# tim-speed/flexdiffuse

Measured on AMD Instinct MI355X. Metric: 512x512 50-step images/sec/node (SD1.5, batch=8/GPU, Linear image guidance), higher is better.
Workload: dtype fp16; 1 GPU; SD1.5 512x512 50-step DDIM + linear image guidance, CFG 8, batch=8/GPU (BASELINE configs[1]); parallelism=seed-sharded x1, preset=sd15, guidance=linear, img2img=False, unet_evaluations_per_image=50, launch=graph, scheduler=ddim

## Files before the change

### flexdiffuse_amd/csrc/norm.hip

```cpp
#include <stdlib.h>

#include "common.h"
#include "gn_slab.h"

#define GN_MAX_CHUNKS 256

__global__ void k_gn_stats(const half_t* __restrict__ x, float* __restrict__ part, int HW, int C,
                           int G, int PL, int pix_per_chunk, int ldx) {
    extern __shared__ float sm[];
    const int b = blockIdx.y, chunk = blockIdx.x;
    const int c8 = C >> 3;
    const int tid = threadIdx.x;
    const int cc = tid % c8, pl = tid / c8;
    const int p0 = chunk * pix_per_chunk;
    const int p1 = min(HW, p0 + pix_per_chunk);
    float s[8], q[8];
#pragma unroll
    for (int k = 0; k < 8; ++k) s[k] = q[k] = 0.f;
    if (pl < PL) {
        const half_t* base = x + ((size_t)b * HW) * ldx + cc * 8;
        int p = p0 + pl;
        uint4 raw[4], nxt[4];
        bool have = p + 3 * PL < p1;
        if (have) {
// ... 402 lines not shown
    FD_CHECK_LAUNCH("k_gn_stats/k_gn_apply");
    return FD_OK;
}

extern "C" int fd_groupnorm_apply_parts_f16(const void* x, int ldx, void* y, const float* gamma, const float* beta, const float* parts,
                                            int chunks, int B, int HW, int C, int G, float eps, int silu, void* stream) {
    FD_PLAN(fd_groupnorm_apply_parts_f16(x, ldx, y, gamma, beta, parts, chunks, B, HW, C, G, eps, silu, fd_s_));
    FD_CHECK_ARG(x && y && gamma && beta && parts, FD_EINVAL, "fd_groupnorm_apply_parts_f16: null pointer");
    FD_CHECK_ARG(B > 0 && HW > 0 && C > 0 && G > 0 && chunks > 0, FD_EINVAL, "fd_groupnorm_apply_parts_f16: bad dims");
    FD_CHECK_ARG(ldx >= C && ldx % 8 == 0 && (uintptr_t)x % 16 == 0 && C % 8 == 0 && C % G == 0 && G <= 64 && C / 8 <= 1024, FD_ESHAPE,
                 "fd_groupnorm_apply_parts_f16: ldx=%d >= C=%d, both multiples of 8, C a multiple of G=%d (G <= 64), x 16-byte aligned", ldx, C, G);
    FD_CHECK_ARG((long long)B * HW * ldx < 0x7fffffffLL, FD_ESHAPE, "fd_groupnorm_apply_parts_f16: tensor too large");
    hipStream_t st = (hipStream_t)stream;
    const int c8 = C / 8;
    int PL = 512 / c8;
    if (PL < 1) PL = 1;
    if (PL > HW) PL = HW;
    const int threads = ((c8 * PL + 63) / 64) * 64;
    int nchunk = 256 / B;
    if (nchunk < 1) nchunk = 1;
    if (nchunk > GN_MAX_CHUNKS) nchunk = GN_MAX_CHUNKS;
    int ppc = fd_cdiv(HW, nchunk);
    if (ppc < PL) ppc = PL;
    nchunk = fd_cdiv(HW, ppc);
    const size_t lds2 = (size_t)2 * threads * sizeof(double) + (size_t)2 * G * sizeof(float);
    fd_prof_begin(FD_FAMILY_GROUPNORM, st, (double)B * HW * C * 4.0, -1.0, fd_tag(13u, B, HW, C, ldx));
    hipLaunchKernelGGL(k_gn_apply, dim3(nchunk, B), dim3(threads), lds2, st, (const half_t*)x, (half_t*)y, parts, gamma, beta, HW, C, G,
                       chunks, PL, ppc, eps, silu, ldx);
    fd_prof_end(FD_FAMILY_GROUPNORM, st);
    FD_CHECK_LAUNCH("k_gn_apply");
    return FD_OK;
}

template <int VPL, int RPW, bool STATS = false>
__global__ __launch_bounds__(256) void k_layernorm(const half_t* __restrict__ x, void* __restrict__ y,
                                                   const float* __restrict__ gamma,
                                                   const float* __restrict__ beta, int rows, int C,
                                                   int ldx, int ldy, float eps, int out_f32) {
    const int lane = threadIdx.x & 63;
    const int row0 = (blockIdx.x * 4 + (threadIdx.x >> 6)) * RPW;
    if (row0 >= rows) return;
    half8 v[RPW][VPL];
#pragma unroll
    for (int r = 0; r < RPW; ++r) {
        const half_t* xr = x + (size_t)min(row0 + r, rows - 1) * ldx;
#pragma unroll
        for (int i = 0; i < VPL; ++i) {
            const int c = (lane + 64 * i) * 8;
            uint4 raw = make_uint4(0u, 0u, 0u, 0u);
            if (c < C) raw = *reinterpret_cast<const uint4*>(xr + c);
            v[r][i] = *reinterpret_cast<half8*>(&raw);
        }
    }
#pragma unroll
    for (int r = 0; r < RPW; ++r) {
        const int row = row0 + r;
        if (row >= rows) break;
        float sum = 0.f;
#pragma unroll
        for (int i = 0; i < VPL; ++i)
#pragma unroll
            for (int k = 0; k < 8; ++k) sum += (float)v[r][i][k];
        const float mean = fd_wave_sum(sum) / (float)C;
        float sq = 0.f;
#pragma unroll
        for (int i = 0; i < VPL; ++i) {
// ... 180 lines not shown
```

### flexdiffuse_amd/hip.py

```python
from __future__ import annotations

import ctypes
import os
from ctypes import c_char_p, c_double, c_float, c_int, c_int32, c_int64, c_uint64, c_void_p
from typing import Optional

import torch

_HERE = os.path.dirname(os.path.abspath(__file__))
LIB_PATH = os.environ.get('FD_LIB_PATH') or os.path.join(_HERE, 'libflexdiffuse_hip.so')

FD_OK, FD_EINVAL, FD_ESHAPE, FD_EHIP = 0, -1, -2, -3


class FDError(RuntimeError):
    '''HIP runtime failure reported by libflexdiffuse_hip.so (FD_EHIP).'''


class fd_tween_params(ctypes.Structure):
    _fields_ = [('threshold_floor', c_double), ('threshold_mult', c_double),
                ('clustered', c_double), ('max_guidance', c_double),
                ('header_max', c_double), ('order', c_int32), ('reuse', c_int32)]


P = c_void_p
_SIGNATURES = {
    'fd_abi_version': (c_int, []),
    'fd_last_error': (c_char_p, []),
    'fd_device_info': (c_int, [c_int, P, P, P, P, c_int]),
    'fd_prof_enable': (c_int, [c_int]),
    'fd_prof_set_stride': (c_int, [c_int]),
    'fd_prof_collect': (c_int, [c_int, P, P, P]),
    'fd_prof_collect2': (c_int, [c_int, P, P, P, P]),
    'fd_prof_calibrate': (c_int, [c_int, P, P]),
    'fd_prof_drain': (c_int, [P, P, P, P, P, c_int64, P]),
    'fd_guidance_workspace_floats': (c_int64, [c_int, c_int, c_int]),
    'fd_guidance_map': (c_int, [P, P, P, P, P, c_int, c_int, c_int, c_int, c_int, c_int, c_int, P]),
    'fd_guidance_tween': (c_int, [P, P, P, P, P, P, P, P, P, c_int, c_int, c_int, c_int, c_int,
                                  ctypes.POINTER(fd_tween_params), P]),
    'fd_guidance_concept_override': (c_int, [P, P, P, P, P, c_int, c_int, c_int, P]),
    'fd_guidance_header_pull': (c_int, [P, P, c_int, c_int, c_int, P]),
    'fd_gemm_f16': (c_int, [P, P]),
    'fd_gemm_can_emit_row_stats': (c_int, [c_int, c_int, c_int, c_int, c_int]),
    'fd_gemm_plan': (c_int, [c_void_p, c_void_p, c_void_p]),
    'fd_gemm_can_fuse_groupnorm': (c_int, [c_int, c_int, c_int, c_int, c_int]),
    'fd_gemm_gn_parts_chunks': (c_int, [P]),
    'fd_groupnorm_apply_parts_f16': (c_int, [P, c_int, P, P, P, P, c_int, c_int, c_int, c_int, c_int, c_float, c_int, P]),
    'fd_groupnorm_fold_linear_parts_f16': (c_int, [P, c_int, c_int, c_int, c_int, c_int, c_float, P, P, c_int, P, P, P]),
    'fd_attention_f16': (c_int, [P, P]),
    'fd_xattn_image_bytes': (c_int64, [c_int, c_int]),
    'fd_xattn_pack_kv_f16': (c_int, [P, P, P, P, c_int, c_int, c_int, c_int, c_int, c_int, c_int64, c_int64, P]),
    'fd_xattn_q_f16': (c_int, [P, P]),
    'fd_groupnorm_workspace_floats': (c_int64, [c_int, c_int]),
    'fd_groupnorm_nhwc_f16': (c_int, [P, P, P, P, P, c_int, c_int, c_int, c_int, c_float, c_int, P]),
    'fd_groupnorm_nhwc_ld_f16': (c_int, [P, c_int, P, P, P, P, c_int, c_int, c_int, c_int, c_float, c_int, P]),
    'fd_layernorm_f16': (c_int, [P, P, P, P, c_int, c_int, c_int, c_int, c_float, c_int, P]),
    'fd_ln_row_stats_f16': (c_int, [P, P, c_int, c_int, c_int, c_float, P]),
    'fd_ln_finalize_stats_f32': (c_int, [P, P, c_int, c_int, c_int, c_float, P]),
    'fd_groupnorm_fold_linear_f16': (c_int, [P, c_int, P, c_int, c_int, c_int, c_int, c_float, P, P, c_int, P, P, P]),
    'fd_softmax_rows_f16': (c_int, [P, c_int, c_int, c_int, c_float, P]),
    'fd_nchw_f32_to_nhwc_f16': (c_int, [P, P, c_int, c_int, c_int, c_int, c_int, c_float, P]),
    'fd_nhwc_f32_to_nchw_f32': (c_int, [P, P, c_int, c_int, c_int, c_int, c_float, c_float, c_int, P]),
    'fd_im2col_f16': (c_int, [P, P] + [c_int] * 12 + [P]),
    'fd_conv3x3_narrow_f16': (c_int, [P, P, P, P, c_int, P, c_int, c_int, c_int, c_int, c_int, c_int, c_int, c_float, P]),
    'fd_concat_channels_f16': (c_int, [P, P, P, c_int64, c_int, c_int, P]),
    'fd_cfg_ddim_step_f32': (c_int, [P, P, P, c_int, c_int, c_int, c_int, c_int, c_float, c_float,
                                     c_float, c_float, c_float, c_int, c_int, P]),
    'fd_axpby_f32': (c_int, [P, P, P, c_int64, c_float, c_float, c_int, P]),
    'fd_embed_tokens_f16': (c_int, [P, P, P, P, c_int, c_int, c_int, c_int, P]),
    'fd_vit_assemble_f16': (c_int, [P, P, P, P, c_int, c_int, c_int, P]),
    'fd_timestep_embedding_f16': (c_int, [P, c_int, P, c_int, c_int, P]),
    'fd_copy2d_f16': (c_int, [P, c_int, P, c_int, c_int64, c_int, P]),
    'fd_repeat_rows_f16': (c_int, [P, c_int, P, c_int, c_int64, c_int, c_int, P]),
    'fd_plan_create': (c_int, [P]),
    'fd_plan_destroy': (c_int, [P]),
    'fd_plan_record_begin': (c_int, [P]),
    'fd_plan_record_end': (c_int, [P]),
    'fd_plan_size': (c_int, [P, P]),
    'fd_plan_replay': (c_int, [P, P]),
    'fd_region_blend_f32': (c_int, [P, P] + [c_int] * 7 + [c_float, P]),
    'fd_composite_step_f32': (c_int, [P, P, P, P, c_int, c_int, c_int, c_int, c_int, c_int, c_float, c_float,
# ... 183 lines not shown
```

### flexdiffuse_amd/ops.py

```python
from __future__ import annotations

import ctypes
import os
from ctypes import c_float, c_int32, c_int64, c_void_p
from dataclasses import dataclass
from typing import Optional, Tuple

import torch

from . import hip

ACT_NONE, ACT_SILU, ACT_QUICK_GELU, ACT_GELU, ACT_GEGLU = 0, 1, 2, 3, 4
FAMILY_GEMM, FAMILY_ATTENTION, FAMILY_GROUPNORM, FAMILY_OTHER = 0, 1, 2, 3


class fd_gemm_desc(ctypes.Structure):
    _fields_ = [('A', c_void_p), ('W', c_void_p), ('C', c_void_p), ('bias', c_void_p),
                ('bias2', c_void_p), ('residual', c_void_p),
                ('M', c_int32), ('N', c_int32), ('K', c_int32),
                ('lda', c_int32), ('ldw', c_int32), ('ldc', c_int32), ('ldr', c_int32),
                ('ld_bias2', c_int32), ('rows_per_sample', c_int32), ('act', c_int32),
                ('out_f32', c_int32), ('alpha', c_float),
                ('conv', c_int32), ('in_h', c_int32), ('in_w', c_int32), ('in_c', c_int32),
                ('out_h', c_int32), ('out_w', c_int32), ('kh', c_int32), ('kw', c_int32),
# ... 739 lines not shown


_gn_ws = {}
_gn_ws_retired = []


def _gn_workspace(B: int, G: int, dev) -> torch.Tensor:
    n = hip.lib().fd_groupnorm_workspace_floats(B, G)
    key = (dev.index if dev.index is not None else 0, WS_SLOT)
    ws = _gn_ws.get(key)
    if ws is None or ws.numel() < n:
        if ws is not None:
            _gn_ws_retired.append(ws)
        ws = torch.empty(n, dtype=torch.float32, device=dev)
        _gn_ws[key] = ws
    return ws


def groupnorm(x: Act, gamma: torch.Tensor, beta: torch.Tensor, G: int, eps: float,
              silu: bool, parts: Optional['GNParts'] = None) -> Act:
    assert x.t.stride(1) == 1
    out = _empty(tuple(x.t.shape), torch.float16, x.t)
    if parts is not None:
        assert parts.G == G and parts.t.shape == (x.B, parts.chunks, G, 2)
        hip.call('fd_groupnorm_apply_parts_f16', x.t.data_ptr(), x.t.stride(0), out.data_ptr(), gamma.data_ptr(), beta.data_ptr(),
                 parts.t.data_ptr(), parts.chunks, x.B, x.HW, x.C, G, eps, int(silu), hip.stream())
        return Act(out, x.B, x.H, x.W)
    ws = _gn_workspace(x.B, G, x.t.device)
    hip.call('fd_groupnorm_nhwc_ld_f16', x.t.data_ptr(), x.t.stride(0), out.data_ptr(), gamma.data_ptr(),
             beta.data_ptr(), ws.data_ptr(), x.B, x.HW, x.C, G, eps, int(silu), hip.stream())
    return Act(out, x.B, x.H, x.W)


@dataclass
class GNFold:
    wg: torch.Tensor
    biasf: torch.Tensor
    G: int
    eps: float
    N: int
    C: int


def prep_gn_fold(w: torch.Tensor, b: Optional[torch.Tensor], gamma: torch.Tensor, beta: torch.Tensor, G: int, eps: float,
                 dev) -> GNFold:
    w = w.reshape(w.shape[0], -1).float()
    N, C = w.shape
    wg = (w * gamma.float()[None, :]).half()
    biasf = (b.float() if b is not None else torch.zeros(N)) + w @ beta.float()
    return GNFold(wg.contiguous().to(dev), biasf.contiguous().to(dev), G, eps, N, C)


GN_FOLD_MAX_C, GN_FOLD_MAX_G = 48 * 1024 // (16 * 2), 64


def gn_fold_supported(B: int, HW: int, N: int, C: Optional[int] = None, G: int = 32) -> bool:
    mode = os.environ.get('FD_UNET_GN_FOLD', '1')
    C = N if C is None else C
    return (mode != '0' and HW % 256 == 0 and B > 1 and (N * 8 <= HW if mode == '1' else N < HW)
            and C <= GN_FOLD_MAX_C and G <= GN_FOLD_MAX_G)


def gn_fold_linear(x: Act, gf: GNFold, parts: Optional['GNParts'] = None) -> Tuple[torch.Tensor, torch.Tensor]:
    assert x.t.stride(1) == 1 and x.C == gf.C
    wb = _empty((x.B, gf.N, gf.C), torch.float16, x.t)
    bb = _empty((x.B, gf.N), torch.float32, x.t)
# ... 345 lines not shown
```

### flexdiffuse_amd/unet.py

```python
from __future__ import annotations

import os
from types import SimpleNamespace
from typing import Dict, List, Optional

import torch

from . import hip, ops
from .ops import Act
from .weights import SD15_UNET, UNetConfig, unet_param_shapes, unet_up_plan


class _Res:
    def __init__(self, sd, name, dev, temb_off):
        self.n1g, self.n1b = ops.f32(sd[name + '.norm1.weight'], dev), ops.f32(sd[name + '.norm1.bias'], dev)
        self.n2g, self.n2b = ops.f32(sd[name + '.norm2.weight'], dev), ops.f32(sd[name + '.norm2.bias'], dev)
        self.conv1 = ops.prep_conv(sd[name + '.conv1.weight'], sd[name + '.conv1.bias'], dev)
        self.conv2 = ops.prep_conv(sd[name + '.conv2.weight'], sd[name + '.conv2.bias'], dev)
        self.short = None
        self.sc_fused = False
        if name + '.conv_shortcut.weight' in sd:
            w = sd[name + '.conv_shortcut.weight']
            w2 = sd[name + '.conv2.weight']
            if os.environ.get('FD_UNET_SC_FUSE', '1') != '0' and w.shape[1] % 64 == 0 and w2.shape[1] % 64 == 0:
# ... 99 lines not shown
            temb_b.append(sd[name + '.time_emb_proj.bias'])
            self._toff += r.cout
            return r

        attn = lambda name, c: _Attn(sd, name, dev, heads[c], cfg.use_linear_projection, cfg.norm_num_groups)
        self.down: List[dict] = []
        for i, c in enumerate(ch):
            blk = {'res': [], 'attn': [], 'down': None}
            for j in range(cfg.layers_per_block):
                blk['res'].append(res(f'down_blocks.{i}.resnets.{j}'))
                blk['attn'].append(attn(f'down_blocks.{i}.attentions.{j}', c) if cfg.cross_attn[i] else None)
            if i != len(ch) - 1:
                blk['down'] = ops.prep_conv(sd[f'down_blocks.{i}.downsamplers.0.conv.weight'],
                                            sd[f'down_blocks.{i}.downsamplers.0.conv.bias'], dev)
            self.down.append(blk)
        self.mid_res0 = res('mid_block.resnets.0')
        self.mid_attn = attn('mid_block.attentions.0', ch[-1])
        self.mid_res1 = res('mid_block.resnets.1')
        self.up: List[dict] = []
        for i, (skips, c, has_attn, has_up) in enumerate(unet_up_plan(cfg)):
            blk = {'res': [], 'attn': [], 'up': None}
            for j in range(len(skips)):
                blk['res'].append(res(f'up_blocks.{i}.resnets.{j}'))
                blk['attn'].append(attn(f'up_blocks.{i}.attentions.{j}', c) if has_attn else None)
            if has_up:
                blk['up'] = ops.prep_conv(sd[f'up_blocks.{i}.upsamplers.0.conv.weight'],
                                          sd[f'up_blocks.{i}.upsamplers.0.conv.bias'], dev)
                blk['up_ph'] = ops.prep_conv_up_phases(sd[f'up_blocks.{i}.upsamplers.0.conv.weight'],
                                                       sd[f'up_blocks.{i}.upsamplers.0.conv.bias'], dev) \
                    if blk['up'].cin % 64 == 0 and not blk['up'].im2col else None
            self.up.append(blk)
        self.out_g, self.out_b = ops.f32(sd['conv_norm_out.weight'], dev), ops.f32(sd['conv_norm_out.bias'], dev)
        self.conv_out = ops.prep_conv(sd['conv_out.weight'], sd['conv_out.bias'], dev)
        self.temb_all = ops.prep_linear(torch.cat(temb_w, 0), torch.cat(temb_b, 0), dev)
        self.temb_total = self._toff
        self._attn_layers = [a for blk in self.down for a in blk['attn'] if a] + [self.mid_attn] + \
                            [a for blk in self.up for a in blk['attn'] if a]
        self._ctx_key = None
        self._ctx_sched = None
        self.ctx_generation = 0
        self._cat_plan = self._plan_concats()

    def _plan_concats(self) -> List[Optional[int]]:
        skip_c, excluded = [self.conv_in.cout], set()
        for blk in self.down:
            for r in blk['res']:
                skip_c.append(r.cout)
            if blk['down'] is not None:
                if blk['down'].im2col:
                    excluded.add(len(skip_c) - 1)
                skip_c.append(blk['down'].cout)
        plan: List[Optional[int]] = [None] * len(skip_c)
        c, i = self.mid_res1.cout, len(skip_c) - 1
        for blk in self.up:
            for r in blk['res']:
                if i not in excluded and r.conv1.cin == c + skip_c[i] and c % 8 == 0 and skip_c[i] % 8 == 0:
                    plan[i] = c
                c, i = r.cout, i - 1
            if blk['up'] is not None:
                c = blk['up'].cout
        return plan

    def set_attention_slice(self, slice_size):
        self.attention_slice = slice_size

    def to(self, device):
# ... 362 lines not shown
                if blk['down'].im2col:
                    h, pend = ops.conv2d(h, blk['down'], stride=2, out=view), None
                else:
                    h, pend = ops.conv2d(h, blk['down'], stride=2, out=view, gn=self._gn1(seq[nres]), keep=True)
                push(h, buf, ch)
        h, hn = self._res(self.mid_res0, h, temb, xn=pend, next_gn=self._attn_gn(self.mid_attn, h))
        h = self._attn(self.mid_attn, h, xn=hn)
        h, _ = self._res(self.mid_res1, h, temb, out=left(h.B * h.HW, self.mid_res1.cout))
        out_parts = None
        for blk in self.up:
            n = len(blk['res'])
            for j, (r, a) in enumerate(zip(blk['res'], blk['attn'])):
                s, sbuf, sch = skips.pop()
                if sbuf is not None and h.t.data_ptr() == sbuf.data_ptr() and h.C == sch:
                    h = Act(sbuf, h.B, h.H, h.W)
                else:
                    h = Act(ops.concat_channels(ops.contiguous_rows(h.t), ops.contiguous_rows(s.t)), h.B, h.H, h.W)
                last = j == n - 1
                dst = None if (last and blk['up'] is not None) else left(h.B * h.HW, r.cout)
                if a is not None:
                    h, hn = self._res(r, h, temb, next_gn=self._attn_gn(a, h))
                    if last and blk['up'] is None:
                        h, out_parts = self._attn(a, h, out=dst, xn=hn, next_parts=self.G)
                    else:
                        h = self._attn(a, h, out=dst, xn=hn)
                else:
                    h, _ = self._res(r, h, temb, out=dst)
            if blk['up'] is not None:
                dst = left(h.B * h.HW * 4, blk['up'].cout)
                if blk.get('up_ph') is not None and h.t.is_contiguous() and ops.up_phases_supported(h.B * h.HW, blk['up'].cout, blk['up'].cin):
                    h = ops.conv2d_up_phases(h, blk['up_ph'], out=dst)
                else:
                    h = ops.conv2d(h, blk['up'], up=True, out=dst)
        h = ops.groupnorm(h, self.out_g, self.out_b, self.G, 1e-5, True, parts=out_parts)
        return ops.conv2d(h, self.conv_out, out_f32=True).t

    def forward(self, sample, timestep, encoder_hidden_states) -> UNetOutput:
        B, C, H, W = sample.shape
        eps = self.forward_nhwc(sample, timestep, encoder_hidden_states)
        return UNetOutput(sample=ops.nhwc_to_nchw(eps, B, self.cfg.out_channels, H, W))
```

### flexdiffuse_amd/vae.py

```python
from __future__ import annotations

from types import SimpleNamespace
from typing import Dict, Optional

import torch

from . import hip, ops
from .ops import Act
from .weights import SD_VAE, VAEConfig, vae_param_shapes


class _VRes:
    def __init__(self, sd, name, dev):
        self.n1g, self.n1b = ops.f32(sd[name + '.norm1.weight'], dev), ops.f32(sd[name + '.norm1.bias'], dev)
        self.n2g, self.n2b = ops.f32(sd[name + '.norm2.weight'], dev), ops.f32(sd[name + '.norm2.bias'], dev)
        self.conv1 = ops.prep_conv(sd[name + '.conv1.weight'], sd[name + '.conv1.bias'], dev)
        self.conv2 = ops.prep_conv(sd[name + '.conv2.weight'], sd[name + '.conv2.bias'], dev)
        self.short = None
        if name + '.conv_shortcut.weight' in sd:
            w = sd[name + '.conv_shortcut.weight']
            self.short = ops.prep_linear(w.reshape(w.shape[0], w.shape[1]),
                                         sd[name + '.conv_shortcut.bias'], dev)


# ... 31 lines not shown
        if self.device.type != 'cuda':
            raise RuntimeError('flexdiffuse_amd.AutoencoderKL needs a HIP device (no CPU fallback)')
        sd, dev, cfg = state_dict, self.device, config
        needed = [k for k in vae_param_shapes(cfg) if encoder or not k.startswith(('encoder.', 'quant_conv'))]
        missing = [k for k in needed if k not in sd]
        if missing:
            raise KeyError(f'VAE state dict is missing {len(missing)} keys, e.g. {missing[:3]}')
        self.G = cfg.norm_num_groups
        ch = cfg.block_out_channels
        rev = list(reversed(ch))
        L = cfg.latent_channels
        conv = lambda n, **kw: ops.prep_conv(sd[n + '.weight'], sd[n + '.bias'], dev, **kw)
        w = torch.zeros((8, 8)); w[:L, :L] = sd['post_quant_conv.weight'].reshape(L, L)
        b = torch.zeros(8); b[:L] = sd['post_quant_conv.bias']
        self.post_quant = ops.prep_linear(w, b, dev)
        self.d_conv_in = conv('decoder.conv_in', cin_pad=8)
        self.d_mid = (_VRes(sd, 'decoder.mid_block.resnets.0', dev),
                      _VAttn(sd, 'decoder.mid_block.attentions.0', dev),
                      _VRes(sd, 'decoder.mid_block.resnets.1', dev))
        self.d_up = []
        for i in range(len(rev)):
            res = [_VRes(sd, f'decoder.up_blocks.{i}.resnets.{j}', dev)
                   for j in range(cfg.layers_per_block + 1)]
            up = conv(f'decoder.up_blocks.{i}.upsamplers.0.conv') if i != len(rev) - 1 else None
            if up is not None and up.cin % 64 == 0 and not up.im2col:
                n = f'decoder.up_blocks.{i}.upsamplers.0.conv'
                up = (up, ops.prep_conv_up_phases(sd[n + '.weight'], sd[n + '.bias'], dev))
            elif up is not None:
                up = (up, None)
            self.d_up.append((res, up))
        self.d_out_g, self.d_out_b = ops.f32(sd['decoder.conv_norm_out.weight'], dev), \
            ops.f32(sd['decoder.conv_norm_out.bias'], dev)
        self.d_conv_out = conv('decoder.conv_out')
        self.has_encoder = encoder
        if encoder:
            self.e_conv_in = conv('encoder.conv_in', cin_pad=4)
            self.e_down = []
            for i in range(len(ch)):
                res = [_VRes(sd, f'encoder.down_blocks.{i}.resnets.{j}', dev)
                       for j in range(cfg.layers_per_block)]
                dn = conv(f'encoder.down_blocks.{i}.downsamplers.0.conv') if i != len(ch) - 1 else None
                self.e_down.append((res, dn))
            self.e_mid = (_VRes(sd, 'encoder.mid_block.resnets.0', dev),
                          _VAttn(sd, 'encoder.mid_block.attentions.0', dev),
                          _VRes(sd, 'encoder.mid_block.resnets.1', dev))
            self.e_out_g, self.e_out_b = ops.f32(sd['encoder.conv_norm_out.weight'], dev), \
                ops.f32(sd['encoder.conv_norm_out.bias'], dev)
            self.e_conv_out = conv('encoder.conv_out')
            w = sd['quant_conv.weight']
            self.quant = ops.prep_linear(w.reshape(w.shape[0], w.shape[1]), sd['quant_conv.bias'], dev)

    def to(self, device):
        return self

    def _res(self, r: _VRes, x: Act) -> Act:
        h = ops.groupnorm(x, r.n1g, r.n1b, self.G, 1e-6, True)
        h = ops.conv2d(h, r.conv1)
        h = ops.groupnorm(h, r.n2g, r.n2b, self.G, 1e-6, True)
        sc = x.t if r.short is None else ops.gemm(x.t, r.short)
        return ops.conv2d(h, r.conv2, residual=sc)

    def _attn(self, a: _VAttn, x: Act) -> Act:
        B, N, C = x.B, x.HW, x.C
        h = ops.groupnorm(x, a.g, a.b, self.G, 1e-6, False)
        q, k = ops.gemm(h.t, a.q), ops.gemm(h.t, a.k)
        vt = ops.gemm_vt(h.t, a.v, B, N, (N + 7) // 8 * 8)
        s = ops.bgemm(q.view(B, N, C), k.view(B, N, C), alpha=C ** -0.5)
        ops.softmax_rows_(s)
        o = ops.bgemm(s, vt[:, :, :N])
        return Act(ops.gemm(o.view(B * N, C), a.o, residual=x.t), B, x.H, x.W)

    def decode_nhwc(self, z: torch.Tensor, scale: float = 1.0) -> Act:
        hip.require_device(z)
        B, _, hh, ww = z.shape
        up = 2 ** (len(self.cfg.block_out_channels) - 1)
        per_sample = hh * up * ww * up * self.cfg.block_out_channels[0]
        chunk = max(1, getattr(self, 'decode_chunk_elems', 1 << 29) // max(per_sample, 1))
        if B > chunk:
            parts = [self.decode_nhwc(z[i:i + chunk], scale) for i in range(0, B, chunk)]
            return Act(torch.cat([p.t for p in parts]), B, parts[0].H, parts[0].W)
        x = ops.nchw_to_nhwc(z, c_pad=8, scale=scale)
        h = Act(ops.gemm(x.t, self.post_quant), x.B, x.H, x.W)
        h = ops.conv2d(h, self.d_conv_in)
        h = self._res(self.d_mid[0], h)
        h = self._attn(self.d_mid[1], h)
        h = self._res(self.d_mid[2], h)
        for res, up in self.d_up:
            for r in res:
                h = self._res(r, h)
            if up is not None:
                if up[1] is not None and ops.up_phases_supported(h.B * h.HW, up[0].cout, up[0].cin) and h.t.is_contiguous():
                    h = ops.conv2d_up_phases(h, up[1])
                else:
                    h = ops.conv2d(h, up[0], up=True)
        h = ops.groupnorm(h, self.d_out_g, self.d_out_b, self.G, 1e-6, True)
        return ops.conv2d(h, self.d_conv_out, out_f32=True)

    def decode(self, z: torch.Tensor):
        img = self.decode_nhwc(z)
        return SimpleNamespace(sample=ops.nhwc_to_nchw(img.t, img.B, self.cfg.out_channels, img.H, img.W))

    def encode(self, x: torch.Tensor):
        if not self.has_encoder:
            raise RuntimeError('this AutoencoderKL was built without its encoder')
        hip.require_device(x)
        h = ops.conv2d(ops.nchw_to_nhwc(x, c_pad=4), self.e_conv_in)
        for res, dn in self.e_down:
            for r in res:
                h = self._res(r, h)
            if dn is not None:
                h = ops.conv2d(h, dn, stride=2, pad=(0, 0), out_hw=(h.H // 2, h.W // 2))
        h = self._res(self.e_mid[0], h)
        h = self._attn(self.e_mid[1], h)
        h = self._res(self.e_mid[2], h)
        h = ops.groupnorm(h, self.e_out_g, self.e_out_b, self.G, 1e-6, True)
        h = ops.conv2d(h, self.e_conv_out)
        m = ops.gemm(h.t, self.quant, out_f32=True)
        L = self.cfg.latent_channels
        mom = ops.nhwc_to_nchw(m, h.B, 2 * L, h.H, h.W)
        mean, logvar = mom[:, :L].contiguous(), mom[:, L:].clamp(-30.0, 20.0).contiguous()
        return SimpleNamespace(latent_dist=DiagonalGaussian(mean, logvar))
```

### include/flexdiffuse_hip.h

```cpp
#ifndef FLEXDIFFUSE_HIP_H
#define FLEXDIFFUSE_HIP_H

#include <stdint.h>

#ifdef __cplusplus
extern "C" {
#endif

#define FD_OK 0
#define FD_EINVAL (-1)
#define FD_ESHAPE (-2)
#define FD_EHIP (-3)

#define FD_ABI_VERSION 12

int fd_abi_version(void);
const char* fd_last_error(void);
int fd_device_info(int device, int* cu_count, int* clock_khz, int64_t* hbm_bytes,
                   char* arch, int arch_len);

#define FD_FAMILY_GEMM 0
#define FD_FAMILY_ATTENTION 1
#define FD_FAMILY_GROUPNORM 2
#define FD_FAMILY_OTHER 3
// ... 118 lines not shown
int fd_attention_f16(const fd_attention_desc* desc, void* stream);

int64_t fd_xattn_image_bytes(int heads, int head_dim);
int fd_xattn_pack_kv_f16(const void* K, const void* Vt, void* k_image, void* v_image, int samples, int n_keys,
                         int heads, int head_dim, int ldk, int ldvt, int64_t k_sample_stride,
                         int64_t vt_sample_stride, void* stream);
typedef struct fd_xattn_desc {
    const void* x;
    const void* wq;
    const float* bias;
    const float* ln_colsum;
    const float* ln_stats;
    const void* k_image;
    const void* v_image;
    void* out;
    int32_t M, ldx, ldw, ldo;
    int32_t rows_per_sample;
    int32_t n_rep;
    int32_t n_keys, heads, head_dim;
    int32_t ln_stats_parts;
    float ln_fold_eps;
} fd_xattn_desc;
int fd_xattn_q_f16(const fd_xattn_desc* desc, void* stream);

int64_t fd_groupnorm_workspace_floats(int B, int G);
int fd_groupnorm_nhwc_f16(const void* x, void* y, const float* gamma, const float* beta,
                          float* ws, int B, int HW, int C, int G, float eps, int silu,
                          void* stream);
int fd_groupnorm_nhwc_ld_f16(const void* x, int ldx, void* y, const float* gamma, const float* beta,
                             float* ws, int B, int HW, int C, int G, float eps, int silu,
                             void* stream);
int fd_groupnorm_apply_parts_f16(const void* x, int ldx, void* y, const float* gamma, const float* beta, const float* parts,
                                 int chunks, int B, int HW, int C, int G, float eps, int silu, void* stream);
int fd_groupnorm_fold_linear_f16(const void* x, int ldx, float* ws, int B, int HW, int C, int G, float eps,
                                 const void* wg, const float* biasf, int N,
                                 void* w_out, float* bias_out, void* stream);
int fd_groupnorm_fold_linear_parts_f16(const float* parts, int chunks, int B, int HW, int C, int G, float eps,
                                       const void* wg, const float* biasf, int N, void* w_out, float* bias_out, void* stream);
int fd_layernorm_f16(const void* x, void* y, const float* gamma, const float* beta, int rows,
                     int C, int ldx, int ldy, float eps, int out_f32, void* stream);
int fd_ln_row_stats_f16(const void* x, float* stats, int rows, int C, int ldx, float eps, void* stream);
int fd_ln_finalize_stats_f32(const float* partials, float* stats, int M, int N, int n_tiles, float eps, void* stream);
int fd_softmax_rows_f16(void* x, int rows, int N, int ld, float scale, void* stream);

int fd_nchw_f32_to_nhwc_f16(const float* x, void* y, int B, int C, int HW, int rep, int c_pad,
                            float scale, void* stream);
int fd_nhwc_f32_to_nchw_f32(const float* x, float* y, int B, int C, int HW, int ld, float a,
                            float b, int clamp01, void* stream);
int fd_conv3x3_narrow_f16(const float* x, const void* w, const float* bias, void* y, int ldy, void* y2, int ldy2, int rep2,
                          int B, int Cin, int H, int W, int Cout, float scale, void* stream);
int fd_im2col_f16(const void* x, void* y, int B, int Hi, int Wi, int Cin, int Ho, int Wo, int KH,
                  int KW, int stride, int pad_t, int pad_l, int k_pad, void* stream);
int fd_concat_channels_f16(const void* a, const void* b, void* out, int64_t M, int Ca, int Cb,
                           void* stream);
int fd_cfg_ddim_step_f32(float* x, const float* eps_nhwc, float* eps_out, int B, int C, int HW,
                         int ld, int cfg, float guidance, float c1, float c2, float c3, float c4,
                         int v_prediction, int do_step, void* stream);
int fd_axpby_f32(const float* x, const float* y, float* out, int64_t n, float a, float b,
                 int exp_half_x, void* stream);
int fd_embed_tokens_f16(const int64_t* ids, const void* tok_emb, const void* pos_emb, void* out,
                        int B, int L, int D, int vocab, void* stream);
int fd_vit_assemble_f16(const void* patches, const void* cls, const void* pos, void* out, int B,
                        int T, int D, void* stream);
int fd_timestep_embedding_f16(const float* t, int t_stride, void* out, int B, int dim, void* stream);
int fd_copy2d_f16(const void* src, int lds, void* dst, int ldd, int64_t rows, int cols, void* stream);
int fd_repeat_rows_f16(const void* src, int lds, void* dst, int ldd, int64_t rows, int cols, int rep, void* stream);
// ... 60 lines not shown
```

Measured before the change: 10.73 images/sec.

## Fuse final GroupNorm+SiLU into narrow-output 3x3 conv for UNet and VAE

```diff
diff --git a/flexdiffuse_amd/csrc/conv_gn_out.hip b/flexdiffuse_amd/csrc/conv_gn_out.hip
--- /dev/null
+++ b/flexdiffuse_amd/csrc/conv_gn_out.hip
@@ -0,0 +1,207 @@
+#include "common.h"
+#include "gn_slab.h"
+
+#define CGO_R 4
+#define CGO_TW 32
+#define CGO_CK 64
+#define CGO_SW (CGO_TW + 2)
+#define CGO_SP ((CGO_R + 2) * CGO_SW)
+#define CGO_PSTRIDE (CGO_CK * 2 + 16)
+#define CGO_NV ((CGO_SP * (CGO_CK / 8) + 255) / 256)
+#define CGO_WVEC (9 * 2 * 4 * 8)
+#define CGO_NW ((CGO_WVEC + 255) / 256)
+#define CGO_MAX_C 1024
+
+__global__ __launch_bounds__(256) void k_conv3x3_gn_out(const half_t* __restrict__ x, int ldx, const float* __restrict__ part, int nchunk_stats,
+                                                        int nsub, const float* __restrict__ gamma, const float* __restrict__ beta, int G,
+                                                        float eps, int silu, const uint4* __restrict__ wp, const float* __restrict__ bias,
+                                                        float* __restrict__ out, int ldo, int H, int W, int C, int Cout, int vec_out) {
+    __shared__ __align__(16) unsigned char strip[CGO_SP * CGO_PSTRIDE];
+    __shared__ uint4 wl[CGO_WVEC];
+    __shared__ floatx2 scsh[CGO_MAX_C];
+    __shared__ float gst[64 * 2];
+    const int tid = threadIdx.x, b = blockIdx.z;
+    const int y0 = blockIdx.y * CGO_R, x0 = blockIdx.x * CGO_TW;
+    const int nck = (C + CGO_CK - 1) / CGO_CK;
+    const int cv = tid & 7;
+    unsigned goff[CGO_NV];
+    const half_t* xb = x + (size_t)b * H * W * ldx;
+#pragma unroll
+    for (int i = 0; i < CGO_NV; ++i) {
+        const int sp = (tid >> 3) + i * 32;
+        const int r = sp / CGO_SW, c = sp - r * CGO_SW;
+        const int gy = y0 - 1 + r, gx = x0 - 1 + c;
+        const bool ok = sp < CGO_SP && gy >= 0 && gy < H && gx >= 0 && gx < W;
+        goff[i] = ok ? (unsigned)((gy * W + gx) * ldx + cv * 8) : ~0u;
+    }
+    uint4 ra[CGO_NV], rw[CGO_NW];
+    auto issue = [&](int kc) __attribute__((always_inline)) {
+        const int c = kc * CGO_CK + cv * 8;
+#pragma unroll
+        for (int i = 0; i < CGO_NV; ++i) {
+            ra[i] = make_uint4(0u, 0u, 0u, 0u);
+            if (goff[i] != ~0u && c < C) ra[i] = *reinterpret_cast<const uint4*>(xb + goff[i] + kc * CGO_CK);
+        }
+#pragma unroll
+        for (int i = 0; i < CGO_NW; ++i) {
+            const int v = tid + i * 256;
+            rw[i] = make_uint4(0u, 0u, 0u, 0u);
+            if (v < CGO_WVEC) rw[i] = wp[(size_t)kc * CGO_WVEC + v];
+        }
+    };
+    issue(0);
+    {
+        double* red = reinterpret_cast<double*>(strip);
+        for (int v = tid; v < nsub * G; v += 256) {
+            const int g = v % G, sub = v / G;
+            double s = 0.0, q = 0.0;
+            const float2* src = reinterpret_cast<const float2*>(part) + ((size_t)b * nchunk_stats) * G + g;
+            for (int k = sub; k < nchunk_stats; k += nsub) {
+                const float2 t = src[(size_t)k * G];
+                s += (double)t.x;
+                q += (double)t.y;
+            }
+            red[sub * G + g] = s;
+            red[nsub * G + sub * G + g] = q;
+        }
+        __syncthreads();
+        const int cpg = C / G;
+        if (tid < G) {
+            double s = 0.0, q = 0.0;
+            for (int u = 0; u < nsub; ++u) {
+                s += red[u * G + tid];
+                q += red[nsub * G + u * G + tid];
+            }
+            const double n = (double)H * W * cpg;
+            const double mean = s / n;
+            double var = q / n - mean * mean;
+            if (var < 0.0) var = 0.0;
+            gst[tid * 2 + 0] = (float)mean;
+            gst[tid * 2 + 1] = (float)(1.0 / sqrt(var + (double)eps));
+        }
+        __syncthreads();
+        for (int c = tid; c < C; c += 256) {
+            const int g = c / cpg;
+            const float a = gst[g * 2 + 1] * gamma[c];
+            scsh[c] = floatx2{a, beta[c] - gst[g * 2 + 0] * a};
+        }
+        __syncthreads();
+    }
+    const int lane = tid & 63, wave = tid >> 6;
+    const int ln = lane & 15, kq = lane >> 4;
+    floatx4 acc[2] = {floatx4{0.f, 0.f, 0.f, 0.f}, floatx4{0.f, 0.f, 0.f, 0.f}};
+    const bool row_live = y0 + wave < H;
+    for (int kc = 0; kc < nck; ++kc) {
+        {
+            const int c0 = kc * CGO_CK + cv * 8;
+            float sc[8], sh[8];
+#pragma unroll
+            for (int k = 0; k < 8; ++k) {
+                const floatx2 t = c0 < C ? scsh[c0 + k] : floatx2{0.f, 0.f};
+                sc[k] = t[0];
+                sh[k] = t[1];
+            }
+#pragma unroll
+            for (int i = 0; i < CGO_NV; ++i) {
+                const int sp = (tid >> 3) + i * 32;
+                if (sp >= CGO_SP) continue;
+                uint4 o = make_uint4(0u, 0u, 0u, 0u);
+                if (goff[i] != ~0u && c0 < C) {
+                    const half8 v = *reinterpret_cast<const half8*>(&ra[i]);
+                    half8 h;
+#pragma unroll
+                    for (int k = 0; k < 8; ++k) h[k] = (half_t)gn_act(fmaf((float)v[k], sc[k], sh[k]), silu);
+                    o = *reinterpret_cast<uint4*>(&h);
+                }
+                *reinterpret_cast<uint4*>(strip + sp * CGO_PSTRIDE + cv * 16) = o;
+            }
+#pragma unroll
+            for (int i = 0; i < CGO_NW; ++i) {
+                const int v = tid + i * 256;
+                if (v < CGO_WVEC) wl[v] = rw[i];
+            }
+        }
+        __syncthreads();
+        if (kc + 1 < nck) issue(kc + 1);
+        if (row_live) {
+#pragma unroll
+            for (int tap = 0; tap < 9; ++tap) {
+                const int ky = tap / 3, kx = tap - ky * 3;
+#pragma unroll
+                for (int ks = 0; ks < 2; ++ks) {
+                    uint4 araw = make_uint4(0u, 0u, 0u, 0u);
+                    if (ln < 8) araw = wl[((tap * 2 + ks) * 4 + kq) * 8 + ln];
+                    const half8 a = *reinterpret_cast<const half8*>(&araw);
+#pragma unroll
+                    for (int cg = 0; cg < 2; ++cg) {
+                        const int sp = (wave + ky) * CGO_SW + cg * 16 + ln + kx;
+                        const half8 bv = *reinterpret_cast<const half8*>(strip + sp * CGO_PSTRIDE + ks * 64 + kq * 16);
+                        acc[cg] = __builtin_amdgcn_mfma_f32_16x16x32_f16(a, bv, acc[cg], 0, 0, 0);
+                    }
+                }
+            }
+        }
+        __syncthreads();
+    }
+    if (!row_live || kq * 4 >= Cout) return;
+    const int gy = y0 + wave;
+#pragma unroll
+    for (int cg = 0; cg < 2; ++cg) {
+        const int gx = x0 + cg * 16 + ln;
+        if (gx >= W) continue;
+        float* dst = out + ((size_t)(b * H + gy) * W + gx) * ldo + kq * 4;
+        float v[4];
+#pragma unroll
+        for (int j = 0; j < 4; ++j) v[j] = acc[cg][j] + ((bias && kq * 4 + j < Cout) ? bias[kq * 4 + j] : 0.f);
+        if (vec_out) {
+            *reinterpret_cast<float4*>(dst) = make_float4(v[0], v[1], v[2], v[3]);
+        } else {
+#pragma unroll
+            for (int j = 0; j < 4; ++j)
+                if (kq * 4 + j < Cout) dst[j] = v[j];
+        }
+    }
+}
+
+static int cgo_apply_nsub(int HW, int C, int G) {
+    const int c8 = C / 8;
+    int PL = 512 / c8;
+    if (PL < 1) PL = 1;
+    if (PL > HW) PL = HW;
+    const int threads = ((c8 * PL + 63) / 64) * 64;
+    return threads / G;
+}
+
+extern "C" int fd_conv3x3_gn_out_supported(int C, int Cout, int G, int ldx, int ldo) {
+    return C > 0 && C % 8 == 0 && C <= CGO_MAX_C && G > 0 && G <= 64 && C % G == 0 && Cout >= 1 && Cout <= 8 && ldx >= C && ldx % 8 == 0 &&
+           ldo >= Cout;
+}
+
+extern "C" int64_t fd_conv3x3_gn_out_weight_halves(int C) {
+    return C > 0 ? (int64_t)((C + CGO_CK - 1) / CGO_CK) * CGO_WVEC * 8 : 0;
+}
+
+extern "C" int fd_conv3x3_gn_out_f32(const void* x, int ldx, const float* parts, int chunks, const float* gamma, const float* beta, int G,
+                                     float eps, int silu, const void* w_packed, const float* bias, float* out, int ldo, int B, int H,
+                                     int W, int C, int Cout, void* stream) {
+    FD_PLAN(fd_conv3x3_gn_out_f32(x, ldx, parts, chunks, gamma, beta, G, eps, silu, w_packed, bias, out, ldo, B, H, W, C, Cout, fd_s_));
+    FD_CHECK_ARG(x && parts && gamma && beta && w_packed && out, FD_EINVAL, "fd_conv3x3_gn_out_f32: null pointer");
+    FD_CHECK_ARG(B > 0 && H > 0 && W > 0 && C > 0 && Cout > 0 && G > 0 && chunks > 0, FD_EINVAL, "fd_conv3x3_gn_out_f32: bad dims");
+    FD_CHECK_ARG(fd_conv3x3_gn_out_supported(C, Cout, G, ldx, ldo), FD_ESHAPE,
+                 "fd_conv3x3_gn_out_f32: C=%d (a multiple of 8 and of G=%d <= 64, <= %d), Cout=%d (<= 8), ldx=%d (>= C, a multiple of 8), ldo=%d (>= Cout)",
+                 C, G, CGO_MAX_C, Cout, ldx, ldo);
+    FD_CHECK_ARG(((uintptr_t)x | (uintptr_t)w_packed) % 16 == 0 && (uintptr_t)out % 4 == 0, FD_ESHAPE,
+                 "fd_conv3x3_gn_out_f32: x and w_packed must be 16-byte aligned");
+    FD_CHECK_ARG((long long)B * H * W * ldx < 0x7fffffffLL && (long long)B * H * W < 0x7fffffffLL && B <= 65535 && fd_cdiv(H, CGO_R) <= 65535,
+                 FD_ESHAPE, "fd_conv3x3_gn_out_f32: tensor too large");
+    hipStream_t st = (hipStream_t)stream;
+    const int nsub = cgo_apply_nsub(H * W, C, G);
+    FD_CHECK_ARG(nsub >= 1 && nsub * G <= 1024, FD_ESHAPE, "fd_conv3x3_gn_out_f32: statistics combine does not fit");
+    const int vec_out = Cout % 4 == 0 && ldo % 4 == 0 && (uintptr_t)out % 16 == 0;
+    fd_prof_begin(FD_FAMILY_GEMM, st, 2.0 * B * H * W * Cout * 9.0 * C, -1.0, fd_tag(31u, B, H * W, C, Cout));
+    hipLaunchKernelGGL(k_conv3x3_gn_out, dim3(fd_cdiv(W, CGO_TW), fd_cdiv(H, CGO_R), B), dim3(256), 0, st, (const half_t*)x, ldx, parts,
+                       chunks, nsub, gamma, beta, G, eps, silu, (const uint4*)w_packed, bias, out, ldo, H, W, C, Cout, vec_out);
+    fd_prof_end(FD_FAMILY_GEMM, st);
+    FD_CHECK_LAUNCH("k_conv3x3_gn_out");
+    return FD_OK;
+}
diff --git a/flexdiffuse_amd/csrc/norm.hip b/flexdiffuse_amd/csrc/norm.hip
--- a/flexdiffuse_amd/csrc/norm.hip
+++ b/flexdiffuse_amd/csrc/norm.hip
@@ -458,6 +458,32 @@
     return FD_OK;
 }
 
+extern "C" int fd_groupnorm_stats_chunks(int B, int HW, int C) {
+    if (B <= 0 || HW <= 0 || C <= 0 || C % 8) return 0;
+    int PL, threads, nchunk, ppc;
+    gn_stats_shape(B, HW, C, &PL, &threads, &nchunk, &ppc);
+    return nchunk;
+}
+
+extern "C" int fd_groupnorm_stats_f16(const void* x, int ldx, float* parts, int B, int HW, int C, int G, void* stream) {
+    FD_PLAN(fd_groupnorm_stats_f16(x, ldx, parts, B, HW, C, G, fd_s_));
+    FD_CHECK_ARG(x && parts, FD_EINVAL, "fd_groupnorm_stats_f16: null pointer");
+    FD_CHECK_ARG(B > 0 && HW > 0 && C > 0 && G > 0, FD_EINVAL, "fd_groupnorm_stats_f16: bad dims");
+    FD_CHECK_ARG(ldx >= C && ldx % 8 == 0 && (uintptr_t)x % 16 == 0 && C % 8 == 0 && C % G == 0 && G <= 64 && C / 8 <= 1024, FD_ESHAPE,
+                 "fd_groupnorm_stats_f16: ldx=%d >= C=%d, both multiples of 8, C a multiple of G=%d (G <= 64), x 16-byte aligned", ldx, C, G);
+    FD_CHECK_ARG((long long)B * HW * ldx < 0x7fffffffLL && B <= 65535, FD_ESHAPE, "fd_groupnorm_stats_f16: tensor too large");
+    int PL, threads, nchunk, ppc;
+    gn_stats_shape(B, HW, C, &PL, &threads, &nchunk, &ppc);
+    const size_t lds = (size_t)PL * C * 2 * sizeof(float);
+    FD_CHECK_ARG(lds <= 64 * 1024, FD_ESHAPE, "fd_groupnorm_stats_f16: stats LDS too large");
+    hipStream_t st = (hipStream_t)stream;
+    fd_prof_begin(FD_FAMILY_GROUPNORM, st, (double)B * HW * C * 2.0, -1.0, fd_tag(14u, B, HW, C, ldx));
+    hipLaunchKernelGGL(k_gn_stats, dim3(nchunk, B), dim3(threads), lds, st, (const half_t*)x, parts, HW, C, G, PL, ppc, ldx);
+    fd_prof_end(FD_FAMILY_GROUPNORM, st);
+    FD_CHECK_LAUNCH("k_gn_stats");
+    return FD_OK;
+}
+
 template <int VPL, int RPW, bool STATS = false>
 __global__ __launch_bounds__(256) void k_layernorm(const half_t* __restrict__ x, void* __restrict__ y,
                                                    const float* __restrict__ gamma,
diff --git a/flexdiffuse_amd/hip.py b/flexdiffuse_amd/hip.py
--- a/flexdiffuse_amd/hip.py
+++ b/flexdiffuse_amd/hip.py
@@ -47,6 +47,12 @@
     'fd_gemm_gn_parts_chunks': (c_int, [P]),
     'fd_groupnorm_apply_parts_f16': (c_int, [P, c_int, P, P, P, P, c_int, c_int, c_int, c_int, c_int, c_float, c_int, P]),
     'fd_groupnorm_fold_linear_parts_f16': (c_int, [P, c_int, c_int, c_int, c_int, c_int, c_float, P, P, c_int, P, P, P]),
+    'fd_groupnorm_stats_chunks': (c_int, [c_int, c_int, c_int]),
+    'fd_groupnorm_stats_f16': (c_int, [P, c_int, P, c_int, c_int, c_int, c_int, P]),
+    'fd_conv3x3_gn_out_supported': (c_int, [c_int, c_int, c_int, c_int, c_int]),
+    'fd_conv3x3_gn_out_weight_halves': (c_int64, [c_int]),
+    'fd_conv3x3_gn_out_f32': (c_int, [P, c_int, P, c_int, P, P, c_int, c_float, c_int, P, P, P, c_int, c_int, c_int, c_int,
+                                      c_int, c_int, P]),
     'fd_attention_f16': (c_int, [P, P]),
     'fd_xattn_image_bytes': (c_int64, [c_int, c_int]),
     'fd_xattn_pack_kv_f16': (c_int, [P, P, P, P, c_int, c_int, c_int, c_int, c_int, c_int, c_int64, c_int64, P]),
diff --git a/flexdiffuse_amd/ops.py b/flexdiffuse_amd/ops.py
--- a/flexdiffuse_amd/ops.py
+++ b/flexdiffuse_amd/ops.py
@@ -795,6 +795,59 @@
     return Act(out, x.B, x.H, x.W)
 
 
+def groupnorm_stats(x: Act, G: int) -> GNParts:
+    assert x.t.stride(1) == 1
+    chunks = hip.lib().fd_groupnorm_stats_chunks(x.B, x.HW, x.C)
+    if chunks <= 0:
+        raise ValueError(f'groupnorm_stats: C={x.C} must be a multiple of 8')
+    ws = _gn_workspace(x.B, G, x.t.device)
+    hip.call('fd_groupnorm_stats_f16', x.t.data_ptr(), x.t.stride(0), ws.data_ptr(), x.B, x.HW, x.C, G, hip.stream())
+    return GNParts(ws[:x.B * chunks * G * 2].view(x.B, chunks, G, 2), chunks, G)
+
+
+@dataclass
+class GNOutConvW:
+    w: torch.Tensor
+    bias: Optional[torch.Tensor]
+    cout: int
+    cin: int
+
+
+UNET_CONV_OUT_DIRECT = os.environ.get('FD_UNET_CONV_OUT_DIRECT', '1') != '0'
+VAE_CONV_OUT_DIRECT = os.environ.get('FD_VAE_CONV_OUT_DIRECT', '1') != '0'
+
+
+def prep_conv_gn_out(w: torch.Tensor, b: Optional[torch.Tensor], dev) -> Optional[GNOutConvW]:
+    cout, cin, kh, kw = w.shape
+    if (kh, kw) != (3, 3) or cout > 8 or cin % 8 or not hip.lib().fd_conv3x3_gn_out_supported(cin, cout, 1, cin, cout):
+        return None
+    nck = (cin + 63) // 64
+    wp = torch.zeros((8, 3, 3, nck * 64), dtype=torch.float32)
+    wp[:cout, :, :, :cin] = w.permute(0, 2, 3, 1).float()
+    wp = wp.reshape(8, 3, 3, nck, 2, 4, 8).permute(3, 1, 2, 4, 5, 0, 6).contiguous().reshape(-1)
+    assert wp.numel() == hip.lib().fd_conv3x3_gn_out_weight_halves(cin)
+    return GNOutConvW(wp.to(dev, torch.float16).contiguous(), _bias(b, dev), cout, cin)
+
+
+def conv_gn_out_supported(x: Act, w: Optional[GNOutConvW], G: int) -> bool:
+    return (w is not None and x.C == w.cin and x.t.stride(1) == 1 and x.t.data_ptr() % 16 == 0
+            and bool(hip.lib().fd_conv3x3_gn_out_supported(x.C, w.cout, G, x.t.stride(0), _round_up(w.cout, 4))))
+
+
+def conv3x3_gn_out(x: Act, w: GNOutConvW, gamma: torch.Tensor, beta: torch.Tensor, G: int, eps: float, silu: bool,
+                   parts: Optional[GNParts] = None, out: Optional[torch.Tensor] = None) -> Act:
+    if parts is None:
+        parts = groupnorm_stats(x, G)
+    assert parts.G == G and parts.t.shape == (x.B, parts.chunks, G, 2) and x.C == w.cin and x.t.stride(1) == 1
+    M = x.B * x.H * x.W
+    if out is None:
+        out = _empty((M, _round_up(w.cout, 4)), torch.float32, x.t)
+    assert out.shape[0] == M and out.shape[1] >= w.cout and out.stride(1) == 1 and out.dtype == torch.float32
+    hip.call('fd_conv3x3_gn_out_f32', x.t.data_ptr(), x.t.stride(0), parts.t.data_ptr(), parts.chunks, gamma.data_ptr(), beta.data_ptr(),
+             G, eps, int(silu), w.w.data_ptr(), _p(w.bias), out.data_ptr(), out.stride(0), x.B, x.H, x.W, x.C, w.cout, hip.stream())
+    return Act(out, x.B, x.H, x.W)
+
+
 @dataclass
 class GNFold:
     wg: torch.Tensor
diff --git a/flexdiffuse_amd/unet.py b/flexdiffuse_amd/unet.py
--- a/flexdiffuse_amd/unet.py
+++ b/flexdiffuse_amd/unet.py
@@ -155,6 +155,7 @@
             self.up.append(blk)
         self.out_g, self.out_b = ops.f32(sd['conv_norm_out.weight'], dev), ops.f32(sd['conv_norm_out.bias'], dev)
         self.conv_out = ops.prep_conv(sd['conv_out.weight'], sd['conv_out.bias'], dev)
+        self.conv_out_gn = ops.prep_conv_gn_out(sd['conv_out.weight'], sd['conv_out.bias'], dev)
         self.temb_all = ops.prep_linear(torch.cat(temb_w, 0), torch.cat(temb_b, 0), dev)
         self.temb_total = self._toff
         self._attn_layers = [a for blk in self.down for a in blk['attn'] if a] + [self.mid_attn] + \
@@ -583,6 +584,8 @@
                     h = ops.conv2d_up_phases(h, blk['up_ph'], out=dst)
                 else:
                     h = ops.conv2d(h, blk['up'], up=True, out=dst)
+        if ops.UNET_CONV_OUT_DIRECT and ops.conv_gn_out_supported(h, self.conv_out_gn, self.G):
+            return ops.conv3x3_gn_out(h, self.conv_out_gn, self.out_g, self.out_b, self.G, 1e-5, True, parts=out_parts).t
         h = ops.groupnorm(h, self.out_g, self.out_b, self.G, 1e-5, True, parts=out_parts)
         return ops.conv2d(h, self.conv_out, out_f32=True).t
 
diff --git a/flexdiffuse_amd/vae.py b/flexdiffuse_amd/vae.py
--- a/flexdiffuse_amd/vae.py
+++ b/flexdiffuse_amd/vae.py
@@ -87,6 +87,7 @@
         self.d_out_g, self.d_out_b = ops.f32(sd['decoder.conv_norm_out.weight'], dev), \
             ops.f32(sd['decoder.conv_norm_out.bias'], dev)
         self.d_conv_out = conv('decoder.conv_out')
+        self.d_conv_out_gn = ops.prep_conv_gn_out(sd['decoder.conv_out.weight'], sd['decoder.conv_out.bias'], dev)
         self.has_encoder = encoder
         if encoder:
             self.e_conv_in = conv('encoder.conv_in', cin_pad=4)
@@ -148,6 +149,8 @@
                     h = ops.conv2d_up_phases(h, up[1])
                 else:
                     h = ops.conv2d(h, up[0], up=True)
+        if ops.VAE_CONV_OUT_DIRECT and ops.conv_gn_out_supported(h, self.d_conv_out_gn, self.G):
+            return ops.conv3x3_gn_out(h, self.d_conv_out_gn, self.d_out_g, self.d_out_b, self.G, 1e-6, True)
         h = ops.groupnorm(h, self.d_out_g, self.d_out_b, self.G, 1e-6, True)
         return ops.conv2d(h, self.d_conv_out, out_f32=True)
 
diff --git a/include/flexdiffuse_hip.h b/include/flexdiffuse_hip.h
--- a/include/flexdiffuse_hip.h
+++ b/include/flexdiffuse_hip.h
@@ -174,6 +174,13 @@
                              void* stream);
 int fd_groupnorm_apply_parts_f16(const void* x, int ldx, void* y, const float* gamma, const float* beta, const float* parts,
                                  int chunks, int B, int HW, int C, int G, float eps, int silu, void* stream);
+int fd_groupnorm_stats_chunks(int B, int HW, int C);
+int fd_groupnorm_stats_f16(const void* x, int ldx, float* parts, int B, int HW, int C, int G, void* stream);
+int fd_conv3x3_gn_out_supported(int C, int Cout, int G, int ldx, int ldo);
+int64_t fd_conv3x3_gn_out_weight_halves(int C);
+int fd_conv3x3_gn_out_f32(const void* x, int ldx, const float* parts, int chunks, const float* gamma, const float* beta, int G,
+                          float eps, int silu, const void* w_packed, const float* bias, float* out, int ldo, int B, int H, int W,
+                          int C, int Cout, void* stream);
 int fd_groupnorm_fold_linear_f16(const void* x, int ldx, float* ws, int B, int HW, int C, int G, float eps,
                                  const void* wg, const float* biasf, int N,
                                  void* w_out, float* bias_out, void* stream);
```

Measured after the change: 10.76 images/sec (median of 6 runs). Within noise of the previous version (+0.2%).
